# careylab/LocoMouse_cpp

Measured on AMD Instinct MI355X. Metric: frames/sec whole-node + achieved HBM GB/s; 1024×256 gray, 6 templates, higher is better.
Workload: dtype f32

## Files before the change

locomouse_cpp_amd/csrc/lm_kernels.hip:

```cpp
#include <hip/hip_runtime.h>
#include <stdint.h>

#include <type_traits>
#include <utility>

#include "lm_device.h"
#include "lm_introsort.h"

#include "lm_dev_common.h"
#include "lm_corr_narrow.h"
#include "lm_tail_bound.h"
#include "lm_tile_plan.h"



__global__ __launch_bounds__(LM_MM_THREADS) void k_minmax(const uint8_t* const* __restrict__ frame_ptr,
                                                          const uint8_t* __restrict__ bkg, int npix, int s0,
                                                          unsigned* __restrict__ mm) {
  const int slot = s0 + blockIdx.y;
  const lm_gu8* __restrict__ F = as_global(frame_ptr[slot]);
  const int nvec = npix >> 4;
  const int per = (nvec + LM_MM_SPLIT - 1) / LM_MM_SPLIT;
  const int v0 = blockIdx.x * per, v1 = min(nvec, v0 + per);
  const lm_gu4* F4 = reinterpret_cast<const lm_gu4*>(F);
// ... 344 lines not shown
      for (int j = 0; j < 4; ++j) w[j] = __builtin_amdgcn_alignbyte(dd[j + 1], dd[j], sh);
      if (run < 0) {
        const uint32_t r0 = __builtin_bswap32(w[3]), r1 = __builtin_bswap32(w[2]), r2 = __builtin_bswap32(w[1]),
                       r3 = __builtin_bswap32(w[0]);
        w[0] = r0;
        w[1] = r1;
        w[2] = r2;
        w[3] = r3;
      }
    };
    auto emit = [&](int f, const uint32_t (&pw)[4], const LmSlot& sl, int R, int C0, unsigned in_mask, auto gray_c) {
      constexpr bool GRAY = decltype(gray_c)::value;
      uint32_t word[4] = {0, 0, 0, 0};
#pragma unroll
      for (int k = 0; k < LM_INGEST_VEC; ++k) {
        const uint32_t pk = (pw[k >> 2] >> (8 * (k & 3))) & 0xFFu, bk = (bw[k >> 2] >> (8 * (k & 3))) & 0xFFu;
        uint32_t o = lut[f][pk > bk ? pk - bk : 0];
        if (GRAY && in_gray_rect(gk, sl, R, C0 + k)) o = glut[o];
        word[k >> 2] |= o << (8 * (k & 3));
      }
#pragma unroll
      for (int j = 0; j < 4; ++j) word[j] &= byte_keep4((in_mask >> (4 * j)) & 0xFu);
      *reinterpret_cast<uint4*>(ext + (int64_t)(sb + f) * ext_slot_bytes + q) = make_uint4(word[0], word[1], word[2], word[3]);
      if (rng)
        rng[(int64_t)(sb + f) * (ext_slot_bytes / LM_INGEST_VEC) + q / LM_INGEST_VEC] =
            block_range(word[0], word[1]) | block_range(word[2], word[3]) << 16;
      if (flag_chunk) {
        uint32_t ha = 0u, hb = 0u;
#pragma unroll
        for (int j = 0; j < 4; ++j) {
          const uint32_t br = bright_bytes(word[j]);
          ha |= br & ma[j];
          hb |= br & mb[j];
        }
        if (ha) s_fl[f][fr][ta] = 1;
        if (hb) s_fl[f][fr][ta + 1] = 1;
      }
    };

    const int R = sl0.crop_y[v] + K.ext_oy[v] + er, C0 = sl0.crop_x[v] + K.ext_ox[v] + ec;
    if (mapped && (m.y & 3) != 0) {
      run = (m.y & 3) == 1 ? 1 : -1;
      lo = m.x;
      inside = (unsigned)m.y >> 16;
      bw[0] = b4.x;
      bw[1] = b4.y;
      bw[2] = b4.z;
      bw[3] = b4.w;
#pragma unroll
      for (int f = 0; f < LM_INGEST_FB; ++f)
        if (f < nf) {
          uint32_t pw[4];
          run_bytes(d[f % PIPE], pw);
          if (f + PIPE < nf) frame_load(f + PIPE, lo, d[f % PIPE]);
          if (gray_on) emit(f, pw, slots[sb + f], R, C0, inside, std::true_type{});
          else emit(f, pw, sl0, R, C0, inside, std::false_type{});
        }
      continue;
    }
    run = ingest_locate(K, cal, bkg, R, C0, bw, lo, inside);
    if (same && run != 0) {
#pragma unroll
      for (int f = 0; f < PIPE; ++f)
        if (f < nf) frame_load(f, lo, d[f]);
#pragma unroll
      for (int f = 0; f < LM_INGEST_FB; ++f)
        if (f < nf) {
          uint32_t pw[4];
          run_bytes(d[f % PIPE], pw);
          if (f + PIPE < nf) frame_load(f + PIPE, lo, d[f % PIPE]);
          if (gray_on) emit(f, pw, slots[sb + f], R, C0, inside, std::true_type{});
          else emit(f, pw, sl0, R, C0, inside, std::false_type{});
        }
      continue;
    }
    int px = sl0.crop_x[v], py = sl0.crop_y[v];
    for (int f = 0; f < nf; ++f) {
      const int slot = sb + f;
      const LmSlot sl = slots[slot];
      const int Rf = sl.crop_y[v] + K.ext_oy[v] + er;
      const int Cf = sl.crop_x[v] + K.ext_ox[v] + ec;
      if (sl.crop_x[v] != px || sl.crop_y[v] != py) {
        px = sl.crop_x[v];
        py = sl.crop_y[v];
        run = ingest_locate(K, cal, bkg, Rf, Cf, bw, lo, inside);
      }
      const lm_gu8* __restrict__ F = as_global(frame_ptr[slot]);
      uint32_t pw[4] = {0, 0, 0, 0};
      if (run != 0) {
        uint32_t d1[5];
        ingest_run_load(F, lo, d1);
        run_bytes(d1, pw);
      } else {
#pragma unroll
        for (int k = 0; k < LM_INGEST_VEC; ++k)
          if ((inside >> k) & 1u) pw[k >> 2] |= (uint32_t)F[ingest_index(K, cal, Rf, Cf + k)] << (8 * (k & 3));
      }
      if (gray_on) emit(f, pw, sl, Rf, Cf, inside, std::true_type{});
      else emit(f, pw, sl, Rf, Cf, inside, std::false_type{});
    }
  }
  ING_PROF(3)
  if (!fl_band || !tl_list) {
    if (pb && threadIdx.x == 0) {
      pb[4] = clock64();
      pb[15] = wall_clock64();
    }
  }
  if (!fl_band) return;
  __syncthreads();
  for (int i = tid; i < nf * FPB * ftx; i += T) {
    const int f = i / (FPB * ftx), r = (i / ftx) % FPB, tx = i % ftx;
    const int ty = band * FPB + r;
    if (ty >= K.fl_ty[v]) continue;
    const int oh_t = min(LM_FH, K.fl_oh[v] - LM_FH * ty);
    const uint8_t b = s_fl[f][r][tx];
    flags[(int64_t)(sb + f) * K.fl_slot + K.fl_off[v] + ty * ftx + tx] = b;
    if (b && tl_list) {
      s_ent[atomicAdd(&s_n, 1)] = ((uint32_t)(sb + f) << 16) | (uint32_t)(ty * ftx + tx);
      atomicAdd(&s_outs, oh_t * min(LM_FW, K.fl_ow[v] - tx * LM_FW));
    }
  }
  if (!tl_list) return;
  __syncthreads();
  const int G = (int)gridDim.y, c = (int)blockIdx.y * LM_TL_NC / G;
  if (tid == 0) {
    s_base = s_n ? atomicAdd(&tl_cnt[v * LM_TL_NC + c], s_n) : 0;
    if (s_outs) atomicAdd(&tl_cnt[(2 + v) * LM_TL_NC + c], s_outs);
  }
  __syncthreads();
  uint32_t* __restrict__ out = tl_list + (int64_t)v * K.tl_stride +
                               (int64_t)lm_tl_y0(c, G) * LM_INGEST_FB * K.fl_tx[v] * K.fl_ty[v] + s_base;
  for (int p = tid; p < s_n; p += T) out[p] = s_ent[p];
  if (pb && threadIdx.x == 0) {
    pb[4] = clock64();
    pb[15] = wall_clock64();
  }
#undef ING_PROF
}

#ifndef LM_TBW_LD
#define LM_TBW_LD 8
#endif
#ifndef LM_TBW_CV
#define LM_TBW_CV 8
#endif
#ifndef LM_TBW_CR
#define LM_TBW_CR 2
#endif
__global__ __launch_bounds__(LM_TB_THREADS) void k_tile_bound_ref(
    const LmConst* __restrict__ Kp, const uint8_t* __restrict__ ext, int64_t ext_slot_bytes, int s0,
    const double* __restrict__ tbc, const uint8_t* __restrict__ bright, uint8_t* __restrict__ tail_flags,
    int32_t* __restrict__ tt_cnt, uint32_t* __restrict__ tt_list, uint8_t* __restrict__ pt_flags,
    int32_t* __restrict__ pt_cnt, uint32_t* __restrict__ pt_list) {
  const LmConst& K = *Kp;
  extern __shared__ uint8_t tb_lds[];
  __shared__ int s_n[3], s_b[3], s_k[3], s_base[3];
  const int v = (int)blockIdx.y, slot = s0 + (int)blockIdx.x;
  const int T = (int)blockDim.x, tid = (int)threadIdx.x;
  const int ew = K.ext_w[v], eh = K.ext_h[v], nbw = ew / LM_TB_BLK;
  uint8_t* bmax = tb_lds;
  uint8_t* bmin = bmax + eh * nbw;
  if (tid < 3) {
    s_n[tid] = 0;
    s_b[tid] = 0;
    s_k[tid] = 0;
  }
  static_assert(DET_PAW_S == 3 && DET_TAIL_B == 2 && DET_TAIL_S == 5, "three detectors per view, the tail last");
  bool on[3], use[3];
  int y_lo = eh, y_hi = 0, b_lo = nbw, b_hi = 0;
#pragma unroll
  for (int k = 0; k < 3; ++k) {
    const LmDet& D = K.det[3 * v + k];
    on[k] = D.kind != 0 ? tt_cnt != nullptr : pt_cnt != nullptr;
    use[k] = on[k] && K.tb_skip[3 * v + k] != 0;
    if (use[k]) {
      y_lo = min(y_lo, D.in_y);
      y_hi = max(y_hi, D.in_y + D.oh + D.kh - 1);
      b_lo = min(b_lo, D.in_x / LM_TB_BLK);
      b_hi = max(b_hi, (D.in_x + D.ow + D.kw - 1 + LM_TB_BLK - 1) / LM_TB_BLK);
    }
  }
  y_hi = min(y_hi, eh);
  b_hi = min(b_hi, nbw);
  if (y_lo < y_hi && b_lo < b_hi) {
    const uint8_t* __restrict__ vsrc =
        ext + (int64_t)slot * ext_slot_bytes + (v ? (int64_t)K.ext_h[0] * K.ext_w[0] : 0);
    static_assert(LM_TB_BLK == 8, "one 8-byte load per block");
    const int nb = b_hi - b_lo, ne = (y_hi - y_lo) * nb;
    for (int e = tid; e < ne; e += T) {
      const int r = y_lo + e / nb, b = b_lo + e % nb;
      const uint2 p = *reinterpret_cast<const uint2*>(vsrc + (int64_t)r * ew + LM_TB_BLK * b);
      unsigned mx = 0u, mn = 255u;
#pragma unroll
      for (int j = 0; j < LM_TB_BLK; ++j) {
        const unsigned q = ((j < 4 ? p.x : p.y) >> (8 * (j & 3))) & 0xFFu;
        mx = max(mx, q);
        mn = min(mn, q);
      }
      bmax[r * nbw + b] = (uint8_t)mx;
      bmin[r * nbw + b] = (uint8_t)mn;
    }
  }
  __syncthreads();
#pragma unroll
  for (int k = 0; k < 3; ++k) {
    if (!use[k]) continue;
    const LmDet& D = K.det[3 * v + k];
    const int ftx = D.kind != 0 ? K.tt_tx[v] : K.fl_tx[v], rows = D.oh + D.kh - 1;
    uint8_t* rmax = tb_lds + K.tb_rng[3 * v + k];
    uint8_t* rmin = rmax + rows * ftx;
    for (int e = tid; e < rows * ftx; e += T) {
      const int r = e / ftx, tx = e - r * ftx;
      int c0, c1, b0, b1;
      lm_tb_span(tx, D.kw, D.ow, &c0, &c1);
      lm_tb_blocks(D.in_x, c0, c1, &b0, &b1);
      unsigned mx = 0u, mn = 255u;
      for (int b = b0; b < b1; ++b) {
        mx = max(mx, (unsigned)bmax[(D.in_y + r) * nbw + b]);
        mn = min(mn, (unsigned)bmin[(D.in_y + r) * nbw + b]);
      }
      rmax[e] = (uint8_t)mx;
      rmin[e] = (uint8_t)mn;
    }
  }
  __syncthreads();
#pragma unroll
  for (int k = 0; k < 3; ++k) {
    if (!on[k]) continue;
    const int d = 3 * v + k;
    const LmDet& D = K.det[d];
    const bool tail = D.kind != 0;
    const int ftx = tail ? K.tt_tx[v] : K.fl_tx[v], ntile = ftx * (tail ? K.tt_ty[v] : K.fl_ty[v]);
    uint8_t* __restrict__ fl = tail ? tail_flags + (int64_t)slot * K.tt_slot + K.tt_off[v]
                                    : pt_flags + (D.list & 1) * K.pt_plane + (int64_t)slot * K.fl_slot + K.fl_off[v];
    const uint8_t* __restrict__ br = tail ? nullptr : bright + (int64_t)slot * K.fl_slot + K.fl_off[v];
    const uint8_t* rmax = tb_lds + K.tb_rng[d];
    const uint8_t* rmin = rmax + (D.oh + D.kh - 1) * ftx;
    const double* __restrict__ P = tbc + K.tb_off[d];
    int mine = 0, mbr = 0;
    for (int i = tid; i < ntile; i += T) {
      bool keep = br ? br[i] != 0 : true;
      mbr += br && keep ? 1 : 0;
      if (keep && use[k])
        keep = !lm_tb_tile_skip(rmax, rmin, ftx, D.oh, D.kh, i / ftx, i % ftx, P, P + D.kh, K.tb_bias[d]);
      if (keep && use[k] && K.tbr_on[d] != 0)
        keep = !lm_tbr_tile_skip(bmax, bmin, nbw, D.in_y, D.in_x, D.oh, D.ow, D.kh, D.kw, i / ftx, i % ftx,
                                 tbc + K.tbr_off[d], K.tb_bias[d], LM_TB_RH, false);
      fl[i] = keep ? 1 : 0;
      mine += keep ? 1 : 0;
    }
    if (mine) atomicAdd(&s_n[k], mine);
    if (mbr) atomicAdd(&s_b[k], mbr);
  }
  __syncthreads();
  const int G = ((int)gridDim.x + LM_INGEST_FB - 1) / LM_INGEST_FB;
  const int c = ((int)blockIdx.x / LM_INGEST_FB) * LM_TL_NC / G;
  if (tid < 3 && (K.det[3 * v + tid].kind != 0 ? tt_cnt != nullptr : pt_cnt != nullptr)) {
    const LmDet& D = K.det[3 * v + tid];
    int32_t* __restrict__ cnt = D.kind != 0 ? tt_cnt + v * LM_TL_NC : pt_cnt + D.list * LM_TL_NC;
    s_base[tid] = s_n[tid] ? atomicAdd(&cnt[c], s_n[tid]) : 0;
    if (D.kind == 0 && s_b[tid]) atomicAdd(&pt_cnt[(LM_NLIST + D.list) * LM_TL_NC + c], s_b[tid]);
  }
  __syncthreads();
#pragma unroll
  for (int k = 0; k < 3; ++k) {
    if (!on[k]) continue;
    const LmDet& D = K.det[3 * v + k];
    const bool tail = D.kind != 0;
    const int ntile = tail ? K.tt_tx[v] * K.tt_ty[v] : K.fl_tx[v] * K.fl_ty[v];
    const uint8_t* __restrict__ fl = tail ? tail_flags + (int64_t)slot * K.tt_slot + K.tt_off[v]
                                          : pt_flags + (D.list & 1) * K.pt_plane + (int64_t)slot * K.fl_slot + K.fl_off[v];
    uint32_t* __restrict__ out =
        (tail ? tt_list + (int64_t)v * K.tt_stride : pt_list + (int64_t)D.list * K.tl_stride) +
        (int64_t)lm_tl_y0(c, G) * LM_INGEST_FB * ntile + s_base[k];
    for (int i = tid; i < ntile; i += T)
      if (fl[i]) out[atomicAdd(&s_k[k], 1)] = ((uint32_t)slot << 16) | (uint32_t)i;
  }
}

DEV uint32_t range_merge(uint32_t a, uint32_t b) { return lm_tb_range_merge(a, b); }
DEV int wave_append(bool p, int* ctr) {
  const unsigned long long m = __ballot(p);
  if (m == 0ull) return 0;
  const int rank = (int)__builtin_amdgcn_mbcnt_hi((unsigned)(m >> 32), __builtin_amdgcn_mbcnt_lo((unsigned)m, 0u));
  int base = 0;
  if (p && rank == 0) base = atomicAdd(ctr, (int)__popcll(m));
  return __shfl(base, __ffsll((long long)m) - 1) + rank;
}
#ifndef LM_TBW_WPE
#define LM_TBW_WPE 8
#endif
#define TBW_SEL(a) (k == 0 ? a[0] : k == 1 ? a[1] : a[2])
template <bool ROWS, bool NARROW>
__global__ __launch_bounds__(LM_TB_THREADS) __attribute__((amdgpu_waves_per_eu(LM_TBW_WPE, 8))) void k_tile_bound(
    const LmConst* __restrict__ Kp, const uint32_t* __restrict__ rng, int64_t rng_slot, int s0, int nslot,
    const double* __restrict__ tbc, const uint8_t* __restrict__ bright, uint8_t* __restrict__ tail_flags,
    int32_t* __restrict__ tt_cnt, uint32_t* __restrict__ tt_list, uint8_t* __restrict__ pt_flags,
    int32_t* __restrict__ pt_cnt, uint32_t* __restrict__ pt_list, unsigned long long* __restrict__ tbs_fallback,
    const LmNarrowOut nwo) {
  const LmConst& K = *Kp;
  extern __shared__ __attribute__((aligned(16))) uint8_t tbw_lds[];
  __shared__ int s_n[3], s_b[3], s_m[3], s_base[3], s_nw;
  __shared__ int s_c[3][2], s_g[3][2], s_p[3][2];
  if (NARROW && threadIdx.x < 6) {
    s_c[threadIdx.x >> 1][threadIdx.x & 1] = 0;
    s_p[threadIdx.x >> 1][threadIdx.x & 1] = 0;
  }
  const int v = (int)blockIdx.y < K.tbw_nband[0] ? 0 : 1;
  const int band = (int)blockIdx.y - (v ? K.tbw_nband[0] : 0);
  const int slot = s0 + (int)blockIdx.x;
  const int T = (int)blockDim.x, tid = (int)threadIdx.x;
  if (tid < 3) {
    s_n[tid] = 0;
    s_b[tid] = 0;
    s_m[tid] = 0;
  }
  if (tid == 0) s_nw = 0;
  bool on[3], use[3], refine[3], tail[3];
  int t0[3], nt[3], ohb[3], ftx[3], tbase[3];
  uint8_t* fl[3];
  int y_lo = K.ext_h[v], y_hi = 0;
#pragma unroll
  for (int k = 0; k < 3; ++k) {
    const int d = 3 * v + k;
    const LmDet& D = K.det[d];
    tail[k] = D.kind != 0;
    on[k] = tail[k] ? tt_cnt != nullptr : pt_cnt != nullptr;
    use[k] = on[k] && K.tbw_use[d] != 0;
    ftx[k] = tail[k] ? K.tt_tx[v] : K.fl_tx[v];
    int nty;
    ohb[k] = lm_tbw_band(D, tail[k] ? K.tt_ty[v] : K.fl_ty[v], K.tbw_br[v], band, &t0[k], &nty);
    nt[k] = on[k] ? nty * ftx[k] : 0;
    tbase[k] = t0[k] * ftx[k];
    fl[k] = tail[k] ? tail_flags + (int64_t)slot * K.tt_slot + K.tt_off[v]
                    : pt_flags + (D.list & 1) * K.pt_plane + (int64_t)slot * K.fl_slot + K.fl_off[v];
    use[k] = use[k] && nt[k] > 0;
    refine[k] = use[k] && K.tbr_on[d] != 0;
    if (use[k]) {
      y_lo = min(y_lo, D.in_y + LM_FH * t0[k]);
      y_hi = max(y_hi, D.in_y + LM_FH * t0[k] + ohb[k] + D.kh - 1);
    }
  }
  y_hi = min(y_hi, K.ext_h[v]);
  const int nrow = max(0, min(y_hi - y_lo, K.tbw_rows[v]));
  const int nbk = K.tbw_nbk[v], nw = nbk / 2;
  uint32_t* B = reinterpret_cast<uint32_t*>(tbw_lds);
  uint32_t* V = reinterpret_cast<uint32_t*>(tbw_lds + K.tbw_v[v]);
  uint32_t* work = reinterpret_cast<uint32_t*>(tbw_lds + K.tbw_work[v]);
  __syncthreads();
  constexpr int LD = LM_TBW_LD;
  const int ne = nrow * nw, ewq = K.ext_w[v] / LM_INGEST_VEC;
  const uint32_t rc = lm_rcp(max(nw, 1));
  const uint32_t* __restrict__ src = rng + (int64_t)slot * rng_slot +
                                     (v ? (int64_t)K.ext_h[0] * K.ext_w[0] / LM_INGEST_VEC : 0) +
                                     (int64_t)min(y_lo, y_hi) * ewq + K.tbw_blo[v] / 2;
  uint32_t w[LD];
  auto rng_load = [&](int e0) {
#pragma unroll
    for (int u = 0; u < LD; ++u) {
      const int e = e0 + u * T + tid;
      if (e < ne) {
        const int r = lm_div(e, rc);
        w[u] = src[r * ewq + (e - r * nw)];
      }
    }
  };
  auto rng_store = [&](int e0) {
#pragma unroll
    for (int u = 0; u < LD; ++u) {
      const int e = e0 + u * T + tid;
      if (e < ne) B[e] = w[u];
    }
  };
  rng_load(0);
  double pnv[3] = {0.0, 0.0, 0.0};
#pragma unroll
  for (int k = 0; k < 3; ++k)
    if (use[k] && tid < 2 * K.det[3 * v + k].kh) pnv[k] = tbc[K.tb_off[3 * v + k] + tid];
  const uint8_t* __restrict__ br = bright + (int64_t)slot * K.fl_slot + K.fl_off[v];
  const int ntot = nt[0] + nt[1] + nt[2];
  for (int i0 = 0; i0 < ntot; i0 += T) {
    const int i = i0 + tid;
    const bool act = i < ntot;
    const int k = i < nt[0] ? 0 : i < nt[0] + nt[1] ? 1 : 2;
    const int j = i - (k == 0 ? 0 : k == 1 ? nt[0] : nt[0] + nt[1]);
    const bool tl = k == 0 ? tail[0] : k == 1 ? tail[1] : tail[2];
    const int tb = k == 0 ? tbase[0] : k == 1 ? tbase[1] : tbase[2];
    bool cand = act;
    if (act && !tl) {
      cand = br[tb + j] != 0;
      if (!cand) (k == 0 ? fl[0] : k == 1 ? fl[1] : fl[2])[tb + j] = 0;
    }
#pragma unroll
    for (int kk = 0; kk < 3; ++kk) {
      const unsigned long long m = __ballot(cand && !tl && k == kk);
      if (m != 0ull && (tid & 63) == 0) atomicAdd(&s_b[kk], (int)__popcll(m));
    }
    const int pos = wave_append(cand, &s_nw);
    if (cand) work[pos] = (uint32_t)k << 28 | (uint32_t)j;
  }
  rng_store(0);
  for (int e0 = LD * T; e0 < ne; e0 += LD * T) {
    rng_load(e0);
    rng_store(e0);
  }
#pragma unroll
  for (int k = 0; k < 3; ++k)
    if (use[k] && tid < 2 * K.det[3 * v + k].kh) reinterpret_cast<double*>(tbw_lds + K.tbw_pn[3 * v + k])[tid] = pnv[k];
  __syncthreads();
  for (int e = tid; e < (nrow - (LM_TB_H - 1)) * nw; e += T)
    V[e] = range_merge(range_merge(B[e], B[e + nw]), range_merge(B[e + 2 * nw], B[e + 3 * nw]));
  static_assert(LM_TB_H == 4, "four-row windows");
  __syncthreads();
  const uint16_t* B16 = reinterpret_cast<const uint16_t*>(B);
  const uint16_t* V16 = reinterpret_cast<const uint16_t*>(V);
  uint16_t* AL = reinterpret_cast<uint16_t*>(tbw_lds + K.tbw_al[v]);
  const int nvr = max(nrow - (LM_TB_H - 1), 0), als = K.tbw_rows[v];
#pragma unroll
  for (int k = 0; k < 3; ++k) {
    if (!refine[k]) continue;
    const LmDet& D = K.det[3 * v + k];
    const int bl = lm_tbr_block_end(D.in_x, D.ow, D.kw, K.ext_w[v] / LM_TB_BLK) - K.tbw_blo[v] - 1;
    for (int r = tid; r < nvr; r += T) AL[k * als + r] = V16[r * nbk + bl];
  }
#pragma unroll
  for (int k = 0; k < 3; ++k) {
    if (!use[k]) continue;
    const int d = 3 * v + k;
    const LmDet& D = K.det[d];
    uint8_t* wmax = tbw_lds + K.tbw_win[d];
    uint8_t* wmin = wmax + K.tbw_wsz[d];
    const int nent = min(lm_tb_win_rows(ohb[k], D.kh) * ftx[k], K.tbw_wsz[d]);
    const uint32_t rc = K.tbw_inv[d];
    const int yb = D.in_y + LM_FH * t0[k] - y_lo;
    for (int e = tid; e < nent; e += T) {
      const int w = lm_div(e, rc), tx = e - w * ftx[k];
      int r0, nr, c0, c1, b0, b1;
      lm_tb_win_src(ohb[k], D.kh, w, &r0, &nr);
      lm_tb_span(tx, D.kw, D.ow, &c0, &c1);
      lm_tb_blocks(D.in_x, c0, c1, &b0, &b1);
      b0 = max(b0 - K.tbw_blo[v], 0);
      b1 = min(b1 - K.tbw_blo[v], nbk);
      const uint16_t* row = (nr == LM_TB_H ? V16 : B16) + (yb + r0) * nbk;
      const int nrr = nr == LM_TB_H ? 1 : nr;
      unsigned mx = 0u, mn = 255u;
      for (int r = 0; r < nrr; ++r, row += nbk)
        for (int b = b0; b < b1; ++b) {
          const unsigned q = row[b];
          mx = max(mx, q & 0xFFu);
          mn = min(mn, q >> 8);
        }
      wmax[e] = (uint8_t)mx;
      wmin[e] = (uint8_t)mn;
    }
  }
  __syncthreads();
  if (refine[0] || refine[1] || refine[2]) {
    constexpr int CV = LM_TBW_CV;
    const int nv = nvr * nw;
    for (int e0 = 0; e0 < nv; e0 += CV * T) {
      uint32_t pv[CV];
#pragma unroll
      for (int u = 0; u < CV; ++u) {
        const int e = e0 + u * T + tid;
        if (e < nv) {
          const int r = lm_div(e, rc);
          const bool last = e - r * nw == nw - 1;
          pv[u] = lm_tbr_pair_word(V[e], last ? 0u : V[e + 1], last);
        }
      }
      __syncthreads();
#pragma unroll
      for (int u = 0; u < CV; ++u) {
        const int e = e0 + u * T + tid;
        if (e < nv) V[e] = pv[u];
      }
    }
  }
  int kh3[3], win3[3], wsz3[3], pn3[3];
  uint32_t inv3[3];
  double bias3[3];
#pragma unroll
  for (int k = 0; k < 3; ++k) {
    const int d = 3 * v + k;
    kh3[k] = K.det[d].kh;
    win3[k] = K.tbw_win[d];
    wsz3[k] = K.tbw_wsz[d];
    pn3[k] = K.tbw_pn[d];
    inv3[k] = K.tbw_inv[d];
    bias3[k] = K.tb_bias[d];
  }
  const int nwork = s_nw;
  for (int w0 = 0; w0 < nwork; w0 += T) {
    const bool act = w0 + tid < nwork;
    const uint32_t item = act ? work[w0 + tid] : 0u;
    const int k = (int)(item >> 28), j = (int)(item & 0x0FFFFFFFu);
    const int tb = TBW_SEL(tbase);
    bool keep = act;
    if (act && TBW_SEL(use)) {
      const int fx = TBW_SEL(ftx), kh = TBW_SEL(kh3);
      const int ty = lm_div(j, TBW_SEL(inv3)), tx = j - ty * fx;
      const uint8_t* wmax = tbw_lds + TBW_SEL(win3);
      const double* pn = reinterpret_cast<const double*>(tbw_lds + TBW_SEL(pn3));
      keep = !lm_tb_tile_skip_win(wmax, wmax + TBW_SEL(wsz3), fx, kh, lm_tb_win_row0(TBW_SEL(ohb), kh, ty), tx, pn,
                                  pn + kh, TBW_SEL(bias3));
    }
    if (act && !(keep && TBW_SEL(refine))) TBW_SEL(fl)[tb + j] = keep ? 1 : 0;
#pragma unroll
    for (int kk = 0; kk < 3; ++kk) {
      const bool mine = act && keep && k == kk;
      const int pos = wave_append(mine, &s_n[kk]);
      if (mine) reinterpret_cast<uint32_t*>(tbw_lds + K.tbw_ent[3 * v + kk])[pos] = ((uint32_t)slot << 16) | (uint32_t)(tb + j);
    }
  }
  __syncthreads();
  uint32_t* mark = work;
  int nr3[3], ent3[3];
#pragma unroll
  for (int k = 0; k < 3; ++k) {
    nr3[k] = refine[k] ? __builtin_amdgcn_readfirstlane(s_n[k]) : 0;
    ent3[k] = K.tbw_ent[3 * v + k];
  }
  const int nref = nr3[0] + nr3[1] + nr3[2];
  if (nref > 0) {
    for (int t = tid; t < nref; t += T) mark[t] = 0u;
    __syncthreads();
    constexpr int WV = 64;
    const int c1 = (nr3[0] * LM_TB_NBX + WV - 1) / WV, c2 = c1 + (nr3[1] * LM_TB_NBX + WV - 1) / WV,
              c3 = c2 + (nr3[2] * LM_TB_NBX + WV - 1) / WV;
    const uint32_t rcx = lm_rcp(LM_TB_NBX);
    for (int ch = __builtin_amdgcn_readfirstlane(tid / WV); ch < c3; ch += T / WV) {
      const int k = ch < c1 ? 0 : ch < c2 ? 1 : 2;
      const int d = 3 * v + k;
      const LmDet& D = K.det[d];
      const int n = TBW_SEL(nr3), fx = TBW_SEL(ftx), tk0 = TBW_SEL(t0), ohk = TBW_SEL(ohb);
      const int e = (ch - (k == 0 ? 0 : k == 1 ? c1 : c2)) * WV + (tid & (WV - 1));
      const int mb = k == 0 ? 0 : k == 1 ? nr3[0] : nr3[0] + nr3[1];
      const uint32_t* ent = reinterpret_cast<const uint32_t*>(tbw_lds + K.tbw_ent[d]);
      const int kh = D.kh, ng = K.tbr_ng[d], nc = lm_tbr_chunks(ng);
      const double* __restrict__ C = tbc + K.tbr_off[d];
      const double bias = K.tb_bias[d];
      const float* __restrict__ Cf = reinterpret_cast<const float*>(tbc + K.tbs_off[d]);
      const int yb = D.in_y + LM_FH * tk0 - y_lo;
      const int bl0 = lm_tbr_block0(D.in_x, 0) - K.tbw_blo[v];
      const int bendl = lm_tbr_block_end(D.in_x, D.ow, D.kw, K.ext_w[v] / LM_TB_BLK) - K.tbw_blo[v];
      const int nbx = (D.ow + LM_TB_BLK - 1) / LM_TB_BLK;
      if (e >= n * LM_TB_NBX) continue;
      const int t = lm_div(e, rcx);
      const int tile = (int)(ent[t] & 0xFFFFu);
      const int ty = lm_div(tile, K.tbw_inv[d]), tx = tile - ty * fx;
      const int xb = tx * LM_TB_NBX + (e - t * LM_TB_NBX);
      if (xb >= nbx) continue;
      const int tyb = ty - tk0;
      const int nr = min(LM_TB_H, ohk - LM_TB_H * tyb);
      const int row0 = yb + LM_TB_H * tyb, ba0 = bl0 + xb;
      auto level_v = [&](auto rows, auto screen) {
        const uint32_t* pw = V + row0 * nw + (ba0 >> 1);
        const uint16_t* alone = AL + k * als + row0;
        const bool clipped = ba0 + ng == bendl;
        const int jl = (ng - 1) % LM_TBR_GC;
        uint32_t w0, w1, w2, x0 = 0u, x1 = 0u;
        unsigned qn, q = 0u;
        bool lastc = false;
        auto fetch = [&]() {
          w0 = pw[0];
          w1 = pw[1];
          w2 = pw[2];
          qn = *alone;
        };
        fetch();
        if constexpr (decltype(rows)::value > 0) {
          constexpr int NG = decltype(rows)::value;
          auto term = [&](int i, int g, unsigned& M, unsigned& m) {
            if (g == 0) {
              lm_tbr_quad_align(w0, w1, w2, ba0, x0, x1);
              q = qn;
              pw += nw;
              alone += 1;
              fetch();
            }
            lm_tbr_quad_get(x0, x1, g, g == NG - 1 && clipped, q, M, m);
          };
          if constexpr (decltype(screen)::value)
            return lm_tbs_decide(lm_tbs_sum_rows_n<NG>(kh, Cf, K.tbs_bf[d], term), K.tbs_e[d]);
          else
            return lm_tbr_sum_rows_n<NG>(kh, C, bias, term) < 0.0 ? -1 : 1;
        }
        return lm_tbr_sum_negative(kh, ng, C, bias, [&](int i, int g, unsigned& M, unsigned& m) {
          if (g % LM_TBR_GC == 0) {
            const int c = g / LM_TBR_GC;
            lm_tbr_quad_align(w0, w1, w2, ba0, x0, x1);
            q = qn;
            lastc = c == nc - 1;
            pw += lastc ? nw - 2 * (nc - 1) : 2;
            alone += lastc ? 1 : 0;
            fetch();
          }
          lm_tbr_quad_get(x0, x1, g % LM_TBR_GC, lastc && clipped && g % LM_TBR_GC == jl, q, M, m);
        }) ? -1 : 1;
      };
      auto level_b = [&](int rs, int nn) {
        return lm_tbr_sum_negative(kh, ng, C, bias, [&](int i, int g, unsigned& M, unsigned& m) {
          const uint16_t* row = B16 + (row0 + rs + i) * nbk;
          M = 0u;
          m = 255u;
          for (int r = 0; r < nn; ++r, row += nbk) {
            unsigned a, b;
            lm_tbr_pair_range(nullptr, row, ba0 + g, bendl, a, b);
            M = max(M, a);
            m = min(m, b);
          }
        });
      };
      using std::integral_constant;
      using std::false_type;
      using std::true_type;
      bool proven;
      if constexpr (!ROWS) {
        proven = nr == LM_TB_H && level_v(integral_constant<int, 0>{}, false_type{}) < 0;
      } else {
        proven = false;
        if (nr != LM_TB_H) {
        } else if (nc != 1) proven = level_v(integral_constant<int, 0>{}, false_type{}) < 0;
        else {
          int dec = 0;
          if (K.tbs_on[d] != 0) {
            if (ng == 4) dec = level_v(integral_constant<int, 4>{}, true_type{});
            else if (ng == 3) dec = level_v(integral_constant<int, 3>{}, true_type{});
            else if (ng == 2) dec = level_v(integral_constant<int, 2>{}, true_type{});
            else dec = level_v(integral_constant<int, 1>{}, true_type{});
            const unsigned long long und = __ballot(dec == 0);
            if (und != 0ull && (tid & (WV - 1)) == __ffsll((long long)und) - 1)
              atomicAdd(tbs_fallback, (unsigned long long)__popcll(und));
          }
          if (dec == 0) {
            if (ng == 4) dec = level_v(integral_constant<int, 4>{}, false_type{});
            else if (ng == 3) dec = level_v(integral_constant<int, 3>{}, false_type{});
            else if (ng == 2) dec = level_v(integral_constant<int, 2>{}, false_type{});
            else dec = level_v(integral_constant<int, 1>{}, false_type{});
          }
          proven = dec < 0;
        }
      }
      if (!proven && !(LM_TB_RH == LM_TB_H && nr == LM_TB_H)) {
        if (LM_TB_RH == LM_TB_H) {
          proven = level_b(0, nr);
        } else {
          proven = true;
          for (int r = 0; r < nr && proven; ++r) proven = level_b(r, 1);
        }
      }
      if constexpr (NARROW) {
        if (!proven) atomicOr(&mark[mb + t], 1u << (e - t * LM_TB_NBX) | (nr != LM_TB_H ? LM_NW_UNTRIED : 0u));
      } else {
        if (!proven) mark[mb + t] = 1u;
      }
    }
    __syncthreads();
    constexpr int CR = LM_TBW_CR;
    for (int g0 = 0; g0 < nref; g0 += CR * T) {
      uint32_t en[CR], mk[CR];
      int kk[CR];
#pragma unroll
      for (int u = 0; u < CR; ++u) {
        const int i = g0 + u * T + tid;
        const bool act = i < nref;
        const int k = i < nr3[0] ? 0 : i < nr3[0] + nr3[1] ? 1 : 2;
        const int t = i - (k == 0 ? 0 : k == 1 ? nr3[0] : nr3[0] + nr3[1]);
        en[u] = act ? reinterpret_cast<const uint32_t*>(tbw_lds + TBW_SEL(ent3))[t] : 0u;
        mk[u] = act ? mark[i] : 0u;
        const bool kp = mk[u] != 0u;

        kk[u] = kp ? k : -1;
        if (act) TBW_SEL(fl)[en[u] & 0xFFFFu] = kp ? 1 : 0;
      }
      __syncthreads();
#pragma unroll
      for (int u = 0; u < CR; ++u)
#pragma unroll
        for (int k = 0; k < 3; ++k) {
          const bool mine = kk[u] == k;
          const int pos = wave_append(mine, &s_m[k]);
          if (mine) reinterpret_cast<uint32_t*>(tbw_lds + ent3[k])[pos] = en[u];
          if (NARROW && mine) mark[(k == 0 ? 0 : k == 1 ? nr3[0] : nr3[0] + nr3[1]) + pos] = mk[u];
        }
    }
    __syncthreads();
    if (tid < 3) {
      const int k = tid;
      if (TBW_SEL(nr3) > 0) s_n[k] = s_m[k];
    }
  }
  __syncthreads();
  const int G = (nslot + LM_INGEST_FB - 1) / LM_INGEST_FB;
  const int c = ((int)blockIdx.x / LM_INGEST_FB) * LM_TL_NC / G;
  if (tid < 3 && (K.det[3 * v + tid].kind != 0 ? tt_cnt != nullptr : pt_cnt != nullptr)) {
    const LmDet& D = K.det[3 * v + tid];
    int32_t* __restrict__ cnt = D.kind != 0 ? tt_cnt + v * LM_TL_NC : pt_cnt + D.list * LM_TL_NC;
    s_base[tid] = s_n[tid] ? atomicAdd(&cnt[c], s_n[tid]) : 0;
    if (D.kind == 0 && s_b[tid]) atomicAdd(&pt_cnt[(LM_NLIST + D.list) * LM_TL_NC + c], s_b[tid]);
  }
  __syncthreads();
#pragma unroll
  for (int k = 0; k < 3; ++k) {
    if (!on[k] || s_n[k] == 0) continue;
    const LmDet& D = K.det[3 * v + k];
    const int ntile = tail[k] ? K.tt_tx[v] * K.tt_ty[v] : K.fl_tx[v] * K.fl_ty[v];
    const uint32_t* ent = reinterpret_cast<const uint32_t*>(tbw_lds + K.tbw_ent[3 * v + k]);
    uint32_t* __restrict__ out =
        (tail[k] ? tt_list + (int64_t)v * K.tt_stride : pt_list + (int64_t)D.list * K.tl_stride) +
        (int64_t)lm_tl_y0(c, G) * LM_INGEST_FB * ntile + s_base[k];
    for (int p = tid; p < s_n[k]; p += T) out[p] = ent[p];
  }
  if constexpr (NARROW) {
    if (nwo.cnt == nullptr) return;
    bool split[3];
    int mbk[3];
#pragma unroll
    for (int k = 0; k < 3; ++k) {
      split[k] = refine[k] && K.nw_on[3 * v + k] != 0;
      mbk[k] = k == 0 ? 0 : k == 1 ? nr3[0] : nr3[0] + nr3[1];
    }
#pragma unroll
    for (int k = 0; k < 3; ++k) {
      if (!on[k]) continue;
      const int n = s_n[k];
      for (int p0 = 0; p0 < n; p0 += T) {
        const int p = p0 + tid;
        const bool act = p < n, nar = act && split[k] && lm_nw_classify(mark[mbk[k] + p]).narrow != 0;
        const unsigned long long mn = __ballot(nar), mw = __ballot(act && !nar);
        if ((tid & 63) == 0) {
          if (mn != 0ull) atomicAdd(&s_c[k][1], (int)__popcll(mn));
          if (mw != 0ull) atomicAdd(&s_c[k][0], (int)__popcll(mw));
        }
      }
    }
    __syncthreads();
    if (tid < 6 && on[tid >> 1]) {
      const int k = tid >> 1, cls = tid & 1, d = 3 * v + k;
      const LmDet& D = K.det[d];
      int32_t* __restrict__ cnt = nwo.cnt + (cls ? LM_NW_CNT_N + d * LM_TL_NC
                                                 : D.kind != 0 ? LM_NW_CNT_TTW + v * LM_TL_NC : LM_NW_CNT_PTW + D.list * LM_TL_NC);
      s_g[k][cls] = s_c[k][cls] ? atomicAdd(&cnt[c], s_c[k][cls]) : 0;
    }
    __syncthreads();
#pragma unroll
    for (int k = 0; k < 3; ++k) {
      if (!on[k]) continue;
      const int n = s_n[k];
      const LmDet& D = K.det[3 * v + k];
      const int ntile = tail[k] ? K.tt_tx[v] * K.tt_ty[v] : K.fl_tx[v] * K.fl_ty[v];
      const uint32_t* ent = reinterpret_cast<const uint32_t*>(tbw_lds + K.tbw_ent[3 * v + k]);
      const int64_t lo = tail[k] ? (int64_t)v * K.tt_stride : (int64_t)D.list * K.tl_stride;
      const int64_t so = (int64_t)lm_tl_y0(c, G) * LM_INGEST_FB * ntile;
      uint32_t* __restrict__ wout = (tail[k] ? nwo.ttw_list : nwo.ptw_list) + lo + so + s_g[k][0];
      unsigned long long* __restrict__ nout = nwo.n_list + (tail[k] ? (int64_t)LM_NLIST * K.tl_stride : 0) + lo + so + s_g[k][1];
      for (int p0 = 0; p0 < n; p0 += T) {
        const int p = p0 + tid;
        const bool act = p < n;
        const LmNwClass cl = act && split[k] ? lm_nw_classify(mark[mbk[k] + p]) : LmNwClass{0, 0, 0};
        const bool nar = cl.narrow != 0;
        const int pn = wave_append(nar, &s_p[k][1]);
        if (nar) nout[pn] = lm_nw_entry(ent[p], cl.first, cl.count);
        const int pw = wave_append(act && !nar, &s_p[k][0]);
        if (act && !nar) wout[pw] = ent[p];
      }
    }
  }
}
#undef TBW_SEL

#include "lm_corr.h"

#include "lm_cc.h"

DEV float key_score(unsigned long long k) { return __uint_as_float(~(unsigned)(k >> 32)); }
DEV unsigned key_lo(unsigned long long k) { return (unsigned)(k & 0xFFFFFFFFu); }
#ifndef LM_TAIL_THREADS
#define LM_TAIL_THREADS 256
#endif
#define LM_TAIL_SEGS 15

struct TailLayout {
  int rowoff, colc, colm, mask, bm, par, area, key, rs, re, mb, ms, bytes;
};
__host__ __device__ inline TailLayout tail_layout(int TW, int HB, int HS, int cap, int ntc) {
  const int Hm = HB > HS ? HB : HS, nb64 = (TW + 63) / 64;
  const int ntrb = (HB + 31) / 32, ntrs = (HS + 31) / 32;
  TailLayout L;
  int o = 0;
  L.rowoff = o;
  o += 4 * (Hm + 1);
  L.colc = o;
  o += 4 * (TW + 2);
  o = (o + 15) & ~15;
  L.colm = o;
  o += 8 * nb64;
  L.mask = o;
  o += 8 * HB * nb64;
  L.bm = o;
  L.par = o;
  L.area = o + 4 * cap;
  L.key = o + 8 * cap;
  const int bmb = 8 * Hm * (nb64 + 1), ufb = 12 * cap;
  o += bmb > ufb ? bmb : ufb;
  L.rs = o;
  o += 2 * cap;
  L.re = o;
  o += 2 * cap;
  o = (o + 15) & ~15;
  L.mb = o;
  o += 4 * LM_TAIL_SEGS * ntrb * ntc * 3;
  L.ms = o;
  o += 4 * LM_TAIL_SEGS * ntrs * 2;
  L.bytes = o;
  return L;
}

DEV void tail_segment(int rx, int rem, int reg, int* seg, int* sx) {
  if (rx < rem * (reg + 1)) {
    *seg = rx / (reg + 1);
    *sx = *seg * (reg + 1);
  } else {
    *seg = rem + (rx - rem * (reg + 1)) / reg;
    *sx = rem * (reg + 1) + (*seg - rem) * reg;
  }
}

template <bool G, class IX>
DEV void tail_bottom_runs(const CCRuns<IX> S, int R, const int* rowoff, int H, unsigned broot, int nb64,
                          unsigned long long* mask, int* colc, int* s_first, int* s_last) {
  for (int i = threadIdx.x; i < R; i += blockDim.x) {
    if (rld<G>(&S.par[i]) != broot) continue;
    const int y = cc_row_of(rowoff, H, i);
    const int x0 = (int)rld<G>(&S.rs[i]), x1 = (int)rld<G>(&S.re[i]);
    for (int k = x0 >> 6; k <= (x1 >> 6); ++k) {
      const int a = max(x0, 64 * k) - 64 * k, b = min(x1, 64 * k + 63) - 64 * k;
      const unsigned long long bits = (b == 63 ? ~0ull : ((1ull << (b + 1)) - 1)) & ~((1ull << a) - 1);
      atomicOr(&mask[(int64_t)y * nb64 + k], bits);
    }
    atomicAdd(&colc[x0], 1);
    atomicSub(&colc[x1 + 1], 1);
    atomicMin(s_first, x0);
    atomicMax(s_last, x1);
  }
}

template <bool G, class IX>
DEV void tail_bottom_moments(const CCRuns<IX> S, int R, const int* rowoff, int H, unsigned broot, int first, int tw,
                             int rem, int reg, unsigned* mb, int ntrb, int ntc) {
  for (int i = threadIdx.x; i < R; i += blockDim.x) {
    if (rld<G>(&S.par[i]) != broot) continue;
    const int y = cc_row_of(rowoff, H, i);
    const int a = max((int)rld<G>(&S.rs[i]), first) - first, b = min((int)rld<G>(&S.re[i]), first + tw - 1) - first;
    int rx = a;
    while (rx <= b) {
      int seg, sx;
      tail_segment(rx, rem, reg, &seg, &sx);
      const int wseg = seg < rem ? reg + 1 : reg;
      const int end = min(b, sx + wseg - 1);
      for (int l0 = rx - sx; l0 <= end - sx;) {
        const int tx = l0 >> 5, l1 = min(end - sx, 32 * tx + 31);
        const unsigned cnt = (unsigned)(l1 - l0 + 1);
        const unsigned sumx = (unsigned)((l0 + l1 - 64 * tx) * (int)cnt / 2);
        unsigned* t = mb + ((seg * ntrb + (y >> 5)) * ntc + tx) * 3;
        atomicAdd(&t[0], cnt);
        atomicAdd(&t[1], sumx);
        atomicAdd(&t[2], (unsigned)(y & 31) * cnt);
        l0 = l1 + 1;
      }
      rx = end + 1;
    }
  }
}

template <bool G, class IX>
DEV void tail_side_moments(const CCRuns<IX> S, int R, const int* rowoff, int H, unsigned broot, const int* s_tx,
                           unsigned* ms, int ntrs) {
  for (int i = threadIdx.x; i < R; i += blockDim.x) {
    if (rld<G>(&S.par[i]) != broot) continue;
    const int y = cc_row_of(rowoff, H, i);
    const int x0 = (int)rld<G>(&S.rs[i]), x1 = (int)rld<G>(&S.re[i]);
    for (int k = 0; k < LM_TAIL_SEGS; ++k)
      if (s_tx[k] > 0 && s_tx[k] >= x0 && s_tx[k] <= x1) {
        atomicAdd(&ms[(k * ntrs + (y >> 5)) * 2], 1u);
        atomicAdd(&ms[(k * ntrs + (y >> 5)) * 2 + 1], (unsigned)(y & 31));
      }
  }
}

template <bool BIG>
__global__ __launch_bounds__(LM_TAIL_THREADS) void k_tail(const LmConst* __restrict__ Kp, int s0,
                                                          const uint8_t* __restrict__ tailbin, int64_t tailbin_slot_bytes,
                                                          unsigned long long* __restrict__ tailmask,
                                                          unsigned* __restrict__ scratch, LmSlotOut* __restrict__ hdr,
                                                          long long* __restrict__ prof, uint8_t* __restrict__ ws,
                                                          int64_t ws_slot, const unsigned long long* __restrict__ keys,
                                                          const int32_t* __restrict__ n_pos) {
  extern __shared__ __attribute__((aligned(16))) uint8_t smt_lds[];
#define TAIL_PROF(k) \
  if (prof && threadIdx.x == 0) prof[blockIdx.x * 16 + (k)] = clock64();
  TAIL_PROF(0)
  if (prof && threadIdx.x == 0) prof[blockIdx.x * 16 + 14] = wall_clock64();
  const LmConst& K = *Kp;
  const int slot = s0 + blockIdx.x;
  uint8_t* smt = BIG ? ws + (int64_t)slot * ws_slot : smt_lds;
  const int TW = K.tail_w, HB = K.tail_hb, HS = K.tail_hs, nb64 = (TW + 63) / 64;
  const int cap = BIG ? 0 : K.tail_cap, ntc = K.tail_ntc, ntrb = (HB + 31) / 32, ntrs = (HS + 31) / 32;
  const TailLayout L = tail_layout(TW, HB, HS, cap, ntc);
  int* rowoff = reinterpret_cast<int*>(smt + L.rowoff);
  int* colc = reinterpret_cast<int*>(smt + L.colc);
  unsigned long long* colm = reinterpret_cast<unsigned long long*>(smt + L.colm);
  unsigned long long* mask = reinterpret_cast<unsigned long long*>(smt + L.mask);
  unsigned long long* bm = reinterpret_cast<unsigned long long*>(smt + L.bm);
  unsigned* mb = reinterpret_cast<unsigned*>(smt + L.mb);
  unsigned* ms = reinterpret_cast<unsigned*>(smt + L.ms);
  const CCRuns<uint16_t> SL{reinterpret_cast<uint16_t*>(smt + L.rs), reinterpret_cast<uint16_t*>(smt + L.re),
                            reinterpret_cast<unsigned*>(smt + L.par), reinterpret_cast<unsigned*>(smt + L.area),
                            reinterpret_cast<unsigned*>(smt + L.key)};
  const int64_t capg = (int64_t)max(HB, HS) * ((TW + 1) / 2);
  unsigned* gb = scratch + (int64_t)slot * 5 * capg;
  const CCRuns<unsigned> SG{gb, gb + capg, gb + 2 * capg, gb + 3 * capg, gb + 4 * capg};
  __shared__ unsigned long long s_red[LM_TAIL_THREADS / 64];
  __shared__ unsigned s_best;
  __shared__ int s_total, s_first, s_last;
  __shared__ int s_tx[LM_TAIL_SEGS];
  const int tid = threadIdx.x, nt = blockDim.x;
  const bool c8 = K.connectivity == 8;
  const bool lds_ok = TW <= 65535;
  const unsigned long long* __restrict__ binb =
      reinterpret_cast<const unsigned long long*>(tailbin + (int64_t)slot * tailbin_slot_bytes);
  const unsigned long long* __restrict__ bins = binb + (int64_t)HB * nb64;

  for (int i = tid; i < TW + 2; i += nt) colc[i] = 0;
  for (int i = tid; i < HB * nb64; i += nt) mask[i] = 0;
  for (int i = tid; i < LM_TAIL_SEGS * ntrb * ntc * 3; i += nt) mb[i] = 0;
  for (int i = tid; i < LM_TAIL_SEGS * ntrs * 2; i += nt) ms[i] = 0;
  if (tid == 0) {
    s_first = 0x7FFFFFFF;
    s_last = -1;
  }

  cc_bitmap_bits(binb, HB, nb64, nullptr, bm, rowoff);
  TAIL_PROF(1)
  cc_wave0_scan(rowoff, HB, &s_total);
  int R = s_total;
  TAIL_PROF(2)
  const bool gb_b = !(lds_ok && R <= cap);
  if (!gb_b) cc_label<false>(SL, bm, nb64, TW, HB, R, rowoff, c8, s_red, &s_best);
  else cc_label<true>(SG, bm, nb64, TW, HB, R, rowoff, c8, s_red, &s_best);
  const unsigned best_b = s_best;
  TAIL_PROF(3)
  const bool have = best_b != 0xFFFFFFFFu;
  if (have) {
    if (!gb_b) tail_bottom_runs<false>(SL, R, rowoff, HB, best_b, nb64, mask, colc, &s_first, &s_last);
    else tail_bottom_runs<true>(SG, R, rowoff, HB, best_b, nb64, mask, colc, &s_first, &s_last);
  }
  __syncthreads();
  const int first = s_first, last = s_last;
  const int tail_width = have ? last - first : 0;
  const int rem = tail_width % LM_TAIL_SEGS, reg = (tail_width - rem) / LM_TAIL_SEGS;
  if (have) {
    if (!gb_b) tail_bottom_moments<false>(SL, R, rowoff, HB, best_b, first, tail_width, rem, reg, mb, ntrb, ntc);
    else tail_bottom_moments<true>(SG, R, rowoff, HB, best_b, first, tail_width, rem, reg, mb, ntrb, ntc);
  }
  if (tid < 64) {
    const int lane = tid;
    int carry = 0;
    for (int k = 0; k < nb64; ++k) {
      const int x = 64 * k + lane;
      int inc = x < TW ? colc[x] : 0;
      for (int o = 1; o < 64; o <<= 1) {
        const int t = __shfl_up(inc, o);
        if (lane >= o) inc += t;
      }
      const unsigned long long b = __ballot(x < TW && carry + inc > 0);
      if (lane == 0) colm[k] = b;
      carry += __shfl(inc, 63);
    }
  }
  __syncthreads();
  TAIL_PROF(4)
  unsigned long long* __restrict__ tm = tailmask + (int64_t)slot * HB * nb64;
  for (int i = tid; i < HB * nb64; i += nt) tm[i] = mask[i];
  for (int feat = 0; feat < LM_NFEAT; ++feat) {
    const LmDet& D = K.det[feat == 0 ? DET_PAW_B : DET_SNOUT_B];
    const unsigned long long* __restrict__ src = keys + (int64_t)slot * K.keys_per_slot + K.list_off[feat];
    const int n = n_pos[slot * LM_NLIST + feat];
    int keep = 0;
    for (int k = tid; k < n && !keep; k += nt) {
      const unsigned idx = key_lo(src[k]);
      const int y = idx / D.ow, x = idx - y * D.ow;
      keep = !(x < TW && y < HB && ((mask[y * nb64 + (x >> 6)] >> (x & 63)) & 1));
    }
    keep = __syncthreads_or(keep);
    if (tid == 0) hdr[slot].bottom_kept[feat] = keep != 0;
  }

  cc_bitmap_bits(bins, HS, nb64, colm, bm, rowoff);
  TAIL_PROF(5)
  cc_wave0_scan(rowoff, HS, &s_total);
  R = s_total;
  const bool gb_s = !(lds_ok && R <= cap);
  if (!gb_s) cc_label<false>(SL, bm, nb64, TW, HS, R, rowoff, c8, s_red, &s_best);
  else cc_label<true>(SG, bm, nb64, TW, HS, R, rowoff, c8, s_red, &s_best);
  const unsigned best_s = s_best;
  TAIL_PROF(6)

  if (tid < LM_TAIL_SEGS) {
    const int i = tid;
    int tx_ = -1, ty_ = -1;
    if (have) {
      const int sx = first + (i < rem ? i * (reg + 1) : rem * (reg + 1) + (i - rem) * reg);
      const int wseg = i < rem ? reg + 1 : reg;
      double m00 = 0, m10 = 0, m01 = 0;
      const double s = 1. / 255;
      const int nc = (wseg + 31) >> 5;
      for (int ty = 0; ty < ntrb; ++ty)
        for (int tx = 0; tx < nc; ++tx) {
          const unsigned* t = mb + ((i * ntrb + ty) * ntc + tx) * 3;
          const double mom0 = (double)(255u * t[0]) * s;
          const double mom1 = (double)(255u * t[1]) * s;
          const double mom2 = (double)(255u * t[2]) * s;
          const double xm = (double)(tx * 32) * mom0, ym = (double)(ty * 32) * mom0;
          m00 += mom0;
          m10 += mom1 + xm;
          m01 += mom2 + ym;
        }
      if (m00 > 0) {
        tx_ = (int)(m10 / m00) + sx;
        ty_ = (int)(m01 / m00) + 0;
      }
    }
    s_tx[i] = tx_;
    hdr[slot].tail[i] = tx_;
    hdr[slot].tail[LM_TAIL_SEGS + i] = ty_;
  }
  __syncthreads();
  TAIL_PROF(7)
  if (best_s != 0xFFFFFFFFu) {
    if (!gb_s) tail_side_moments<false>(SL, R, rowoff, HS, best_s, s_tx, ms, ntrs);
    else tail_side_moments<true>(SG, R, rowoff, HS, best_s, s_tx, ms, ntrs);
  }
  __syncthreads();
  TAIL_PROF(8)
  if (tid < LM_TAIL_SEGS) {
    const int i = tid;
    int tz = -1;
    if (s_tx[i] > 0) {
      double m00 = 0, m01 = 0;
      const double s = 1. / 255;
      for (int ty = 0; ty < ntrs; ++ty) {
        const double mom0 = (double)(255u * ms[(i * ntrs + ty) * 2]) * s;
        const double mom2 = (double)(255u * ms[(i * ntrs + ty) * 2 + 1]) * s;
        const double ym = (double)(ty * 32) * mom0;
        m00 += mom0;
        m01 += mom2 + ym;
      }
      if (m00 > 0) tz = (int)(m01 / m00) + 0;
    }
    hdr[slot].tail[2 * LM_TAIL_SEGS + i] = tz;
  }
  if (prof && threadIdx.x == 0) {
    prof[blockIdx.x * 16 + 9] = clock64();
    prof[blockIdx.x * 16 + 13] = R;
    prof[blockIdx.x * 16 + 15] = wall_clock64();
  }
#undef TAIL_PROF
}
// ... 1503 lines not shown
```

Measured before the change: 988,800.

## Use one wave per detector for narrow tile-bound list compaction and emission

In the NARROW variant of k_tile_bound, the block-wide compaction pass through LDS, which relied on shared counters and several __syncthreads barriers, is removed. Each detector is now handled by a single wave. That wave classifies its entries, writes the tile flags, counts narrow and wide entries with ballots, reserves global list space with lane-0 atomics, and writes the outputs using mbcnt-based offsets. The non-narrow path keeps its old behaviour. The aim is to cut block barriers, LDS atomics and the extra pass over the compacted list. In exchange only three waves do the final work, and the wide entries are no longer written to the plain tt/pt lists in the narrow path; only their counts are updated.

```diff
diff --git a/locomouse_cpp_amd/csrc/lm_kernels.hip b/locomouse_cpp_amd/csrc/lm_kernels.hip
--- a/locomouse_cpp_amd/csrc/lm_kernels.hip
+++ b/locomouse_cpp_amd/csrc/lm_kernels.hip
@@ -670,11 +670,6 @@
   const LmConst& K = *Kp;
   extern __shared__ __attribute__((aligned(16))) uint8_t tbw_lds[];
   __shared__ int s_n[3], s_b[3], s_m[3], s_base[3], s_nw;
-  __shared__ int s_c[3][2], s_g[3][2], s_p[3][2];
-  if (NARROW && threadIdx.x < 6) {
-    s_c[threadIdx.x >> 1][threadIdx.x & 1] = 0;
-    s_p[threadIdx.x >> 1][threadIdx.x & 1] = 0;
-  }
   const int v = (int)blockIdx.y < K.tbw_nband[0] ? 0 : 1;
   const int band = (int)blockIdx.y - (v ? K.tbw_nband[0] : 0);
   const int slot = s0 + (int)blockIdx.x;
@@ -682,7 +677,7 @@
   if (tid < 3) {
     s_n[tid] = 0;
     s_b[tid] = 0;
-    s_m[tid] = 0;
+    if (!NARROW) s_m[tid] = 0;
   }
   if (tid == 0) s_nw = 0;
   bool on[3], use[3], refine[3], tail[3];
@@ -1026,114 +1021,126 @@
       }
     }
     __syncthreads();
-    constexpr int CR = LM_TBW_CR;
-    for (int g0 = 0; g0 < nref; g0 += CR * T) {
-      uint32_t en[CR], mk[CR];
-      int kk[CR];
-#pragma unroll
-      for (int u = 0; u < CR; ++u) {
-        const int i = g0 + u * T + tid;
-        const bool act = i < nref;
-        const int k = i < nr3[0] ? 0 : i < nr3[0] + nr3[1] ? 1 : 2;
-        const int t = i - (k == 0 ? 0 : k == 1 ? nr3[0] : nr3[0] + nr3[1]);
-        en[u] = act ? reinterpret_cast<const uint32_t*>(tbw_lds + TBW_SEL(ent3))[t] : 0u;
-        mk[u] = act ? mark[i] : 0u;
-        const bool kp = mk[u] != 0u;
-
-        kk[u] = kp ? k : -1;
-        if (act) TBW_SEL(fl)[en[u] & 0xFFFFu] = kp ? 1 : 0;
+    if constexpr (!NARROW) {
+      constexpr int CR = LM_TBW_CR;
+      for (int g0 = 0; g0 < nref; g0 += CR * T) {
+        uint32_t en[CR], mk[CR];
+        int kk[CR];
+#pragma unroll
+        for (int u = 0; u < CR; ++u) {
+          const int i = g0 + u * T + tid;
+          const bool act = i < nref;
+          const int k = i < nr3[0] ? 0 : i < nr3[0] + nr3[1] ? 1 : 2;
+          const int t = i - (k == 0 ? 0 : k == 1 ? nr3[0] : nr3[0] + nr3[1]);
+          en[u] = act ? reinterpret_cast<const uint32_t*>(tbw_lds + TBW_SEL(ent3))[t] : 0u;
+          mk[u] = act ? mark[i] : 0u;
+          const bool kp = mk[u] != 0u;
+
+          kk[u] = kp ? k : -1;
+          if (act) TBW_SEL(fl)[en[u] & 0xFFFFu] = kp ? 1 : 0;
+        }
+        __syncthreads();
+#pragma unroll
+        for (int u = 0; u < CR; ++u)
+#pragma unroll
+          for (int k = 0; k < 3; ++k) {
+            const bool mine = kk[u] == k;
+            const int pos = wave_append(mine, &s_m[k]);
+            if (mine) reinterpret_cast<uint32_t*>(tbw_lds + ent3[k])[pos] = en[u];
+          }
       }
       __syncthreads();
-#pragma unroll
-      for (int u = 0; u < CR; ++u)
-#pragma unroll
-        for (int k = 0; k < 3; ++k) {
-          const bool mine = kk[u] == k;
-          const int pos = wave_append(mine, &s_m[k]);
-          if (mine) reinterpret_cast<uint32_t*>(tbw_lds + ent3[k])[pos] = en[u];
-          if (NARROW && mine) mark[(k == 0 ? 0 : k == 1 ? nr3[0] : nr3[0] + nr3[1]) + pos] = mk[u];
-        }
-    }
-    __syncthreads();
-    if (tid < 3) {
-      const int k = tid;
-      if (TBW_SEL(nr3) > 0) s_n[k] = s_m[k];
-    }
-  }
-  __syncthreads();
+      if (tid < 3) {
+        const int k = tid;
+        if (TBW_SEL(nr3) > 0) s_n[k] = s_m[k];
+      }
+    }
+  }
   const int G = (nslot + LM_INGEST_FB - 1) / LM_INGEST_FB;
   const int c = ((int)blockIdx.x / LM_INGEST_FB) * LM_TL_NC / G;
-  if (tid < 3 && (K.det[3 * v + tid].kind != 0 ? tt_cnt != nullptr : pt_cnt != nullptr)) {
-    const LmDet& D = K.det[3 * v + tid];
-    int32_t* __restrict__ cnt = D.kind != 0 ? tt_cnt + v * LM_TL_NC : pt_cnt + D.list * LM_TL_NC;
-    s_base[tid] = s_n[tid] ? atomicAdd(&cnt[c], s_n[tid]) : 0;
-    if (D.kind == 0 && s_b[tid]) atomicAdd(&pt_cnt[(LM_NLIST + D.list) * LM_TL_NC + c], s_b[tid]);
-  }
-  __syncthreads();
-#pragma unroll
-  for (int k = 0; k < 3; ++k) {
-    if (!on[k] || s_n[k] == 0) continue;
-    const LmDet& D = K.det[3 * v + k];
-    const int ntile = tail[k] ? K.tt_tx[v] * K.tt_ty[v] : K.fl_tx[v] * K.fl_ty[v];
-    const uint32_t* ent = reinterpret_cast<const uint32_t*>(tbw_lds + K.tbw_ent[3 * v + k]);
-    uint32_t* __restrict__ out =
-        (tail[k] ? tt_list + (int64_t)v * K.tt_stride : pt_list + (int64_t)D.list * K.tl_stride) +
-        (int64_t)lm_tl_y0(c, G) * LM_INGEST_FB * ntile + s_base[k];
-    for (int p = tid; p < s_n[k]; p += T) out[p] = ent[p];
-  }
   if constexpr (NARROW) {
-    if (nwo.cnt == nullptr) return;
-    bool split[3];
-    int mbk[3];
+    static_assert(LM_TB_THREADS >= 3 * 64, "a wave per detector of a view");
+    const int k = __builtin_amdgcn_readfirstlane(tid >> 6), lane = tid & 63;
+    if (k >= 3 || !TBW_SEL(on)) return;
+    const int d = 3 * v + k;
+    const LmDet& D = K.det[d];
+    const bool tl = D.kind != 0;
+    const int n = __builtin_amdgcn_readfirstlane(s_n[k]);
+    const int nb = tl ? 0 : __builtin_amdgcn_readfirstlane(s_b[k]);
+    if (n == 0 && nb == 0) return;
+    const bool rf = TBW_SEL(refine), sp = rf && K.nw_on[d] != 0;
+    const uint32_t* ent = reinterpret_cast<const uint32_t*>(tbw_lds + TBW_SEL(ent3));
+    const uint32_t* mk = mark + (k == 0 ? 0 : k == 1 ? nr3[0] : nr3[0] + nr3[1]);
+    uint8_t* __restrict__ flk = TBW_SEL(fl);
+    uint32_t e = 0u;
+    int cls = 0, fc = 0;
+    auto chunk = [&](int p0, bool flags) {
+      const int p = p0 + lane;
+      cls = 0;
+      if (p < n) {
+        e = ent[p];
+        const uint32_t m = rf ? mk[p] : 0u;
+        const bool kept = !rf || m != 0u;
+        if (flags && rf) flk[e & 0xFFFFu] = kept ? 1 : 0;
+        const LmNwClass cl = sp ? lm_nw_classify(m) : LmNwClass{0, 0, 0};
+        cls = !kept ? 0 : cl.narrow != 0 ? 2 : 1;
+        fc = cl.first | cl.count << 4;
+      }
+    };
+    int cn = 0, cw = 0;
+    for (int p0 = 0; p0 < n; p0 += 64) {
+      chunk(p0, true);
+      cn += (int)__popcll(__ballot(cls == 2));
+      cw += (int)__popcll(__ballot(cls == 1));
+    }
+    int32_t* __restrict__ cnt = tl ? tt_cnt + v * LM_TL_NC : pt_cnt + D.list * LM_TL_NC;
+    int32_t* __restrict__ wcnt = nwo.cnt + (tl ? LM_NW_CNT_TTW + v * LM_TL_NC : LM_NW_CNT_PTW + D.list * LM_TL_NC);
+    int32_t* __restrict__ ncnt = nwo.cnt + LM_NW_CNT_N + d * LM_TL_NC;
+    int gn = 0, gw = 0;
+    if (lane == 0) {
+      if (cn) gn = atomicAdd(&ncnt[c], cn);
+      if (cw) gw = atomicAdd(&wcnt[c], cw);
+      if (cn + cw) atomicAdd(&cnt[c], cn + cw);
+      if (nb) atomicAdd(&pt_cnt[(LM_NLIST + D.list) * LM_TL_NC + c], nb);
+    }
+    if (cn + cw == 0) return;
+    gn = __builtin_amdgcn_readfirstlane(gn);
+    gw = __builtin_amdgcn_readfirstlane(gw);
+    const int ntile = tl ? K.tt_tx[v] * K.tt_ty[v] : K.fl_tx[v] * K.fl_ty[v];
+    const int64_t lo = tl ? (int64_t)v * K.tt_stride : (int64_t)D.list * K.tl_stride;
+    const int64_t so = (int64_t)lm_tl_y0(c, G) * LM_INGEST_FB * ntile;
+    uint32_t* __restrict__ wout = (tl ? nwo.ttw_list : nwo.ptw_list) + lo + so;
+    unsigned long long* __restrict__ nout = nwo.n_list + (tl ? (int64_t)LM_NLIST * K.tl_stride : 0) + lo + so;
+    for (int p0 = 0; p0 < n; p0 += 64) {
+      if (n > 64) chunk(p0, false);
+      const unsigned long long bn = __ballot(cls == 2), bw = __ballot(cls == 1);
+      if (cls == 2)
+        nout[gn + (int)__builtin_amdgcn_mbcnt_hi((unsigned)(bn >> 32), __builtin_amdgcn_mbcnt_lo((unsigned)bn, 0u))] =
+            lm_nw_entry(e, fc & 15, fc >> 4);
+      if (cls == 1)
+        wout[gw + (int)__builtin_amdgcn_mbcnt_hi((unsigned)(bw >> 32), __builtin_amdgcn_mbcnt_lo((unsigned)bw, 0u))] = e;
+      gn += (int)__popcll(bn);
+      gw += (int)__popcll(bw);
+    }
+  } else {
+    __syncthreads();
+    if (tid < 3 && (K.det[3 * v + tid].kind != 0 ? tt_cnt != nullptr : pt_cnt != nullptr)) {
+      const LmDet& D = K.det[3 * v + tid];
+      int32_t* __restrict__ cnt = D.kind != 0 ? tt_cnt + v * LM_TL_NC : pt_cnt + D.list * LM_TL_NC;
+      s_base[tid] = s_n[tid] ? atomicAdd(&cnt[c], s_n[tid]) : 0;
+      if (D.kind == 0 && s_b[tid]) atomicAdd(&pt_cnt[(LM_NLIST + D.list) * LM_TL_NC + c], s_b[tid]);
+    }
+    __syncthreads();
 #pragma unroll
     for (int k = 0; k < 3; ++k) {
-      split[k] = refine[k] && K.nw_on[3 * v + k] != 0;
-      mbk[k] = k == 0 ? 0 : k == 1 ? nr3[0] : nr3[0] + nr3[1];
-    }
-#pragma unroll
-    for (int k = 0; k < 3; ++k) {
-      if (!on[k]) continue;
-      const int n = s_n[k];
-      for (int p0 = 0; p0 < n; p0 += T) {
-        const int p = p0 + tid;
-        const bool act = p < n, nar = act && split[k] && lm_nw_classify(mark[mbk[k] + p]).narrow != 0;
-        const unsigned long long mn = __ballot(nar), mw = __ballot(act && !nar);
-        if ((tid & 63) == 0) {
-          if (mn != 0ull) atomicAdd(&s_c[k][1], (int)__popcll(mn));
-          if (mw != 0ull) atomicAdd(&s_c[k][0], (int)__popcll(mw));
-        }
-      }
-    }
-    __syncthreads();
-    if (tid < 6 && on[tid >> 1]) {
-      const int k = tid >> 1, cls = tid & 1, d = 3 * v + k;
-      const LmDet& D = K.det[d];
-      int32_t* __restrict__ cnt = nwo.cnt + (cls ? LM_NW_CNT_N + d * LM_TL_NC
-                                                 : D.kind != 0 ? LM_NW_CNT_TTW + v * LM_TL_NC : LM_NW_CNT_PTW + D.list * LM_TL_NC);
-      s_g[k][cls] = s_c[k][cls] ? atomicAdd(&cnt[c], s_c[k][cls]) : 0;
-    }
-    __syncthreads();
-#pragma unroll
-    for (int k = 0; k < 3; ++k) {
-      if (!on[k]) continue;
-      const int n = s_n[k];
+      if (!on[k] || s_n[k] == 0) continue;
       const LmDet& D = K.det[3 * v + k];
       const int ntile = tail[k] ? K.tt_tx[v] * K.tt_ty[v] : K.fl_tx[v] * K.fl_ty[v];
       const uint32_t* ent = reinterpret_cast<const uint32_t*>(tbw_lds + K.tbw_ent[3 * v + k]);
-      const int64_t lo = tail[k] ? (int64_t)v * K.tt_stride : (int64_t)D.list * K.tl_stride;
-      const int64_t so = (int64_t)lm_tl_y0(c, G) * LM_INGEST_FB * ntile;
-      uint32_t* __restrict__ wout = (tail[k] ? nwo.ttw_list : nwo.ptw_list) + lo + so + s_g[k][0];
-      unsigned long long* __restrict__ nout = nwo.n_list + (tail[k] ? (int64_t)LM_NLIST * K.tl_stride : 0) + lo + so + s_g[k][1];
-      for (int p0 = 0; p0 < n; p0 += T) {
-        const int p = p0 + tid;
-        const bool act = p < n;
-        const LmNwClass cl = act && split[k] ? lm_nw_classify(mark[mbk[k] + p]) : LmNwClass{0, 0, 0};
-        const bool nar = cl.narrow != 0;
-        const int pn = wave_append(nar, &s_p[k][1]);
-        if (nar) nout[pn] = lm_nw_entry(ent[p], cl.first, cl.count);
-        const int pw = wave_append(act && !nar, &s_p[k][0]);
-        if (act && !nar) wout[pw] = ent[p];
-      }
+      uint32_t* __restrict__ out =
+          (tail[k] ? tt_list + (int64_t)v * K.tt_stride : pt_list + (int64_t)D.list * K.tl_stride) +
+          (int64_t)lm_tl_y0(c, G) * LM_INGEST_FB * ntile + s_base[k];
+      for (int p = tid; p < s_n[k]; p += T) out[p] = ent[p];
     }
   }
 }
```

New measurement: 1.011 million, median of 6. +2.3%, better.
